# maggieHao/multi_modal_transformers_TokenMerge

Measured on NVIDIA B200. Metric: ToMe-transformer train samples/sec, higher is better.
Workload: dtype bf16

## Files before the change

multi_modal_transformers_tokenmerge_b200/csrc/attn_bwd.cu:

```cuda
#include <float.h>

#include "attn_meta.cuh"
#include "common.cuh"
#include "host_util.h"

namespace tome {

int check_attn_desc(const tome_attn_desc_t* d, const char* who);
int attn_generic_bwd(const tome_attn_desc_t* d, const tome_attn_grad_strides_t* gs, const void* q, const void* k, const void* v,
                     const void* out, const float* lse, const void* dout, void* dq, void* dk, void* dv, cudaStream_t stream);

constexpr int AB_D = 64;
constexpr int AB_THREADS = 192;
constexpr int DKT_SOFTMAX_WARPS = 8;
constexpr int DKT_THREADS = 320;
constexpr uint32_t AB_TMEM_COLS = 256;
constexpr int AB_MSLOTS = 3;

struct AttnBwdParams {
  int batch, tokens, heads, tp;
  float scale, scale_log2;
  const uint8_t* gid;
  const int32_t* pos;
  const uint8_t* meta;
  int store_ds;

  const float* size;
  const float* lse2;
  const float* delta;
  const uint8_t* keep_q;
  const uint8_t* keep_k;
  float inv_keep;
  __nv_bfloat16* dq; long long dq_bs, dq_ts;
  __nv_bfloat16* dk; long long dk_bs, dk_ts;
  __nv_bfloat16* dv; long long dv_bs, dv_ts;
  float* cs;
  long long cs_ld;
  int cs_q, cs_k, cs_v, n_t128;
};

__device__ __forceinline__ void warp_arrive(uint64_t* bar, int lane) {
  __syncwarp();
  if (lane == 0) mbar_arrive(bar);
}

__device__ __forceinline__ void ab_store_tile(uint8_t* stage, float* part, uint32_t tm_row, int rows_valid, __nv_bfloat16* gtile,
                                              long long row_stride, float* colsum_out, int bar) {
  const int tid = threadIdx.x & 127, row = tid, warp = tid >> 5, lane = tid & 31;
// ... 41 lines not shown
  const long long total = (long long)B * Tp * H * 8;
  if (idx < total) {
    const int ch = (int)(idx & 7);
    const long long r = idx >> 3;
    const int h = (int)(r % H);
    const long long bt = r / H;
    const int t = (int)(bt % Tp), b = (int)(bt / Tp);
    float s = 0.f;
    if (t < T) {
      const uint4 ov = __ldg(reinterpret_cast<const uint4*>(o + b * o_bs + t * o_ts + h * AB_D + ch * 8));
      const uint4 dv = __ldg(reinterpret_cast<const uint4*>(dout + b * do_bs + t * do_ts + h * AB_D + ch * 8));
      s = bf16_lo(ov.x) * bf16_lo(dv.x) + bf16_hi(ov.x) * bf16_hi(dv.x) + bf16_lo(ov.y) * bf16_lo(dv.y) +
          bf16_hi(ov.y) * bf16_hi(dv.y) + bf16_lo(ov.z) * bf16_lo(dv.z) + bf16_hi(ov.z) * bf16_hi(dv.z) +
          bf16_lo(ov.w) * bf16_lo(dv.w) + bf16_hi(ov.w) * bf16_hi(dv.w);
    }
    s += __shfl_xor_sync(0xffffffffu, s, 1);
    s += __shfl_xor_sync(0xffffffffu, s, 2);
    s += __shfl_xor_sync(0xffffffffu, s, 4);
    if (ch == 0) {
      const long long w = ((long long)b * H + h) * Tp + t;
      delta[w] = s;
      lse2[w] = t < T ? lse[((long long)b * H + h) * T + t] * 1.4426950408889634f : INFINITY;
    }
  }
}

constexpr int DKV_BK = 128;
constexpr int DKV_BQ = 64;
static_assert(DKV_BQ == ATTN_META_TILE, "query tiles and metadata tiles must coincide");
constexpr int DKV_KV_BYTES = DKV_BK * AB_D * 2;
constexpr int DKV_Q_BYTES = DKV_BQ * AB_D * 2;
constexpr int DKV_PT_BYTES = DKV_BK * DKV_BQ * 2;
constexpr int DKV_META_SLOT = 1280 + ATTN_DROP_TILE_BYTES;

constexpr int DKT_SMEM = 2 * DKV_KV_BYTES + 2 * 2 * DKV_Q_BYTES + 2 * DKV_PT_BYTES + AB_MSLOTS * DKV_META_SLOT + 256 + 1024;

template <bool DROP>
__global__ void __launch_bounds__(DKT_THREADS, 2)
attn_bwd_dkdv_ts_kernel(const __grid_constant__ CUtensorMap tm_q, const __grid_constant__ CUtensorMap tm_k,
                        const __grid_constant__ CUtensorMap tm_v, const __grid_constant__ CUtensorMap tm_do,
                        const __grid_constant__ CUtensorMap tm_ds, const AttnBwdParams p) {
  extern __shared__ uint8_t smem_raw[];
  uint8_t* smem = smem_raw + ((1024u - (smem_u32(smem_raw) & 1023u)) & 1023u);
  uint8_t* s_k = smem;
  uint8_t* s_v = s_k + DKV_KV_BYTES;
  uint8_t* s_qdo = s_v + DKV_KV_BYTES;
  uint8_t* s_dst = s_qdo + 2 * 2 * DKV_Q_BYTES;
  uint8_t* s_meta = s_dst + 2 * DKV_PT_BYTES;
  uint64_t* bars = reinterpret_cast<uint64_t*>(s_meta + AB_MSLOTS * DKV_META_SLOT);
  uint64_t* kv_full = bars;
  uint64_t* q_full = bars + 1;
  uint64_t* q_empty = bars + 3;
  uint64_t* s_full = bars + 5;
  uint64_t* dp_full = bars + 6;
  uint64_t* s_free = bars + 7;
  uint64_t* ps_ready = bars + 8;
  uint64_t* pd_free = bars + 9;
  uint64_t* meta_full = bars + 10;
  uint64_t* meta_empty = bars + 13;
  uint64_t* ds_stored = bars + 16;
  uint32_t* tmem_slot = reinterpret_cast<uint32_t*>(bars + 18);

  const int warp = threadIdx.x >> 5, lane = threadIdx.x & 31;
  const int kt = blockIdx.x, h = blockIdx.y, b = blockIdx.z;
  const int T = p.tokens;
  const int n_q = (T + DKV_BQ - 1) / DKV_BQ;
  const bool has_mask = p.gid != nullptr;

  if (threadIdx.x == 0) {
    mbar_init(kv_full, 1);
    for (int i = 0; i < 2; ++i) {
      mbar_init(&q_full[i], 1);
      mbar_init(&q_empty[i], 1);
    }
    mbar_init(s_full, 1);
    mbar_init(dp_full, 1);
    mbar_init(s_free, DKT_SOFTMAX_WARPS);
    mbar_init(ps_ready, DKT_SOFTMAX_WARPS);
    mbar_init(pd_free, 1);
    mbar_init(&ds_stored[0], 1);
    mbar_init(&ds_stored[1], 1);
    for (int i = 0; i < AB_MSLOTS; ++i) {
      mbar_init(&meta_full[i], 1);
      mbar_init(&meta_empty[i], DKT_SOFTMAX_WARPS);
    }
    fence_barrier_init();
  }
  if (warp == 8 && lane == 0) {
    tma_prefetch_desc(&tm_q);
    tma_prefetch_desc(&tm_k);
    tma_prefetch_desc(&tm_v);
    tma_prefetch_desc(&tm_do);
  }
  if (warp == 9) tmem_alloc(tmem_slot, AB_TMEM_COLS);
  tc_fence_before();
  __syncthreads();
  tc_fence_after();
  const uint32_t tmem_base = *tmem_slot;
  const uint32_t tm_st = tmem_base, tm_dpt = tmem_base + 64, tm_dk = tmem_base + 128, tm_dv = tmem_base + 192;
  auto tm_dsa = [&](int k) { return tm_dpt + (uint32_t)((k >> 1) * 32 + (k & 1) * 8); };
  auto tm_pa = [&](int k) { return tm_dpt + (uint32_t)((k >> 1) * 32 + 16 + (k & 1) * 8); };

  if (warp == 8) {
    if (lane == 0) {
      mbar_expect_tx(kv_full, 2 * DKV_KV_BYTES);
      tma_load_3d(s_k, &tm_k, kv_full, h * AB_D, kt * DKV_BK, b);
      tma_load_3d(s_v, &tm_v, kv_full, h * AB_D, kt * DKV_BK, b);
      const float* lse_row = p.lse2 + ((size_t)b * p.heads + h) * p.tp;
      const float* del_row = p.delta + ((size_t)b * p.heads + h) * p.tp;
      const uint8_t* meta_b = p.meta + (size_t)b * n_q * ATTN_META_BYTES;
      for (int i = 0; i < n_q; ++i) {
        const int ms = i % AB_MSLOTS;
        uint8_t* slot = s_meta + ms * DKV_META_SLOT;
        mbar_wait(&meta_empty[ms], ((i / AB_MSLOTS) & 1) ^ 1);
        mbar_expect_tx(&meta_full[ms], (has_mask ? 1280u : 512u) + (DROP ? ATTN_DROP_TILE_BYTES : 0));
        if constexpr (DROP) bulk_g2s(slot + 1280, p.keep_k + ((size_t)kt * n_q + i) * ATTN_DROP_TILE_BYTES, ATTN_DROP_TILE_BYTES, &meta_full[ms]);
        bulk_g2s(slot, lse_row + i * DKV_BQ, 256, &meta_full[ms]);
        bulk_g2s(slot + 256, del_row + i * DKV_BQ, 256, &meta_full[ms]);
        if (has_mask) bulk_g2s(slot + 512, meta_b + (size_t)i * ATTN_META_BYTES + ATTN_META_OFF_POS, 768, &meta_full[ms]);
        const int st = i & 1;
        mbar_wait(&q_empty[st], ((i >> 1) & 1) ^ 1);
        mbar_expect_tx(&q_full[st], 2 * DKV_Q_BYTES);
        tma_load_3d(s_qdo + st * 2 * DKV_Q_BYTES, &tm_q, &q_full[st], h * AB_D, i * DKV_BQ, b);
        tma_load_3d(s_qdo + st * 2 * DKV_Q_BYTES + DKV_Q_BYTES, &tm_do, &q_full[st], h * AB_D, i * DKV_BQ, b);
      }
    }
  } else if (warp == 9) {
    if (lane == 0) {
      constexpr uint32_t idesc_s = make_idesc_bf16(DKV_BK, DKV_BQ, false, false);
      constexpr uint32_t idesc_g = make_idesc_bf16(DKV_BK, AB_D, false, true);
      const uint32_t ak = smem_u32(s_k), av = smem_u32(s_v);
      mbar_wait(kv_full, 0);
      for (int i = 0; i <= n_q; ++i) {
        if (i < n_q) {
          const int st = i & 1;
          if (i >= 1) {
            mbar_wait(s_free, (i - 1) & 1);
            tc_fence_after();
          }
          mbar_wait(&q_full[st], (i >> 1) & 1);
          tc_fence_after();
          const uint32_t aq = smem_u32(s_qdo + st * 2 * DKV_Q_BYTES);
#pragma unroll
          for (int k = 0; k < AB_D / 16; ++k)
            umma_bf16(tm_st, make_smem_desc(ak + k * 32, 16, 1024), make_smem_desc(aq + k * 32, 16, 1024), idesc_s, k > 0);
          umma_commit(s_full);
        }
        if (i >= 1) {
          mbar_wait(ps_ready, (i - 1) & 1);
          tc_fence_after();
          const int st = (i - 1) & 1;
          const uint32_t aq = smem_u32(s_qdo + st * 2 * DKV_Q_BYTES), ado = aq + DKV_Q_BYTES;
          if (p.store_ds) {
            asm volatile("cp.async.bulk.tensor.3d.global.shared::cta.bulk_group [%0, {%2, %3, %4}], [%1];"
                         ::"l"(&tm_ds), "r"(smem_u32(s_dst + ((i - 1) & 1) * DKV_PT_BYTES)), "r"((i - 1) * DKV_BQ), "r"(kt * DKV_BK), "r"(b * p.heads + h) : "memory");
            asm volatile("cp.async.bulk.commit_group;" ::: "memory");
          }
#pragma unroll
          for (int k = 0; k < DKV_BQ / 16; ++k)
            umma_bf16_ts(tm_dv, tm_pa(k), make_smem_desc(ado + k * 2048, 8192, 1024), idesc_g, (i > 1 || k > 0) ? 1u : 0u);
#pragma unroll
          for (int k = 0; k < DKV_BQ / 16; ++k)
            umma_bf16_ts(tm_dk, tm_dsa(k), make_smem_desc(aq + k * 2048, 8192, 1024), idesc_g, (i > 1 || k > 0) ? 1u : 0u);
          umma_commit(pd_free);
          umma_commit(&q_empty[st]);
        }
        if (i < n_q) {
          const int st = i & 1;
          const uint32_t ado = smem_u32(s_qdo + st * 2 * DKV_Q_BYTES) + DKV_Q_BYTES;
#pragma unroll
          for (int k = 0; k < AB_D / 16; ++k)
            umma_bf16(tm_dpt, make_smem_desc(av + k * 32, 16, 1024), make_smem_desc(ado + k * 32, 16, 1024), idesc_s, k > 0);
          umma_commit(dp_full);
        }
        if (i >= 2 && p.store_ds) {
          asm volatile("cp.async.bulk.wait_group.read 1;" ::: "memory");
          mbar_arrive(&ds_stored[i & 1]);
        }
      }
      if (p.store_ds) asm volatile("cp.async.bulk.wait_group 0;" ::: "memory");
    }
  } else {
    const int row = (warp & 3) * 32 + lane;
    const int hq = warp >> 2;
    const int kk = kt * DKV_BK + row;
    const uint32_t lane_sel = ((uint32_t)((warp & 3) * 32)) << 16;
    const bool k_valid = kk < T;
    float bias2 = 0.f;
    int gk = 0, pk = 0;
    if (k_valid) {
      if (p.size) bias2 = log2f(p.size[(long long)b * T + kk]);
      if (has_mask) {
        gk = p.gid[(long long)b * T + kk];
        pk = p.pos[(long long)b * T + kk];
      }
    }
    const float2 scale2 = make_float2(p.scale_log2, p.scale_log2), bias22 = make_float2(bias2, bias2);
    const float2 sc2 = make_float2(p.scale, p.scale), ik2 = make_float2(p.inv_keep, p.inv_keep);
    const bool warp_active = kt * DKV_BK + (warp & 3) * 32 < T;
    uint8_t* dst_row0 = s_dst + row * 128;
    for (int i = 0; i < n_q; ++i) {
      const int ms = i % AB_MSLOTS;
      const uint8_t* slot = s_meta + ms * DKV_META_SLOT;
      mbar_wait(&meta_full[ms], (i / AB_MSLOTS) & 1);
      if (!warp_active) {
        mbar_wait(s_full, i & 1);
        tc_fence_before();
        warp_arrive(s_free, lane);
        mbar_wait(dp_full, i & 1);
        if (p.store_ds) {
          uint8_t* dst_row = dst_row0 + (i & 1) * DKV_PT_BYTES;
          if (i >= 2) mbar_wait(&ds_stored[i & 1], ((i - 2) >> 1) & 1);
#pragma unroll
          for (int ch = 0; ch < 4; ++ch) *reinterpret_cast<uint4*>(dst_row + ((hq * 4 + ch) << 4)) = make_uint4(0u, 0u, 0u, 0u);
          fence_proxy_async_smem();
        }
        warp_arrive(&meta_empty[ms], lane);
        tc_fence_before();
        warp_arrive(ps_ready, lane);
        continue;
      }
      uint32_t vw = 0xffffffffu;
      if (has_mask) {
        vw = *reinterpret_cast<const uint32_t*>(slot + 768 + gk * 8 + hq * 4);
        const uint32_t c = *reinterpret_cast<const uint32_t*>(slot + 1024 + gk * 8 + hq * 4);
        if (c) {
          const int* posq = reinterpret_cast<const int*>(slot + 512) + hq * 32;
          for (int q = 0; q < 32; ++q)
            if (((c >> q) & 1u) && pk <= posq[q]) vw |= 1u << q;
        }
      }
      if (!k_valid) vw = 0u;
      uint32_t kb = 0xffffffffu;
      if constexpr (DROP) kb = *reinterpret_cast<const uint32_t*>(slot + 1280 + row * 8 + hq * 4);
      const float4* lse4 = reinterpret_cast<const float4*>(slot) + hq * 8;
      const float4* del4 = reinterpret_cast<const float4*>(slot + 256) + hq * 8;
      uint32_t pe[16];
      mbar_wait(s_full, i & 1);
      tc_fence_after();
      {
        float sv[32];
        tmem_ld_f32x32(tm_st + lane_sel + hq * 32, sv);
        tmem_ld_wait();
        tc_fence_before();
        warp_arrive(s_free, lane);
#pragma unroll
        for (int c4 = 0; c4 < 8; ++c4) {
          const float4 l4 = lse4[c4];
#pragma unroll
          for (int u = 0; u < 2; ++u) {
            const int c = c4 * 4 + 2 * u;
            const float2 lv = u ? make_float2(l4.z, l4.w) : make_float2(l4.x, l4.y);
            float2 t = __ffma2_rn(make_float2(sv[c], sv[c + 1]), scale2, bias22);
            t = __fadd2_rn(t, make_float2(-lv.x, -lv.y));
            float2 e = make_float2(fast_exp2(t.x), fast_exp2(t.y));
            e.x = ((vw >> c) & 1u) ? e.x : 0.f;
            e.y = ((vw >> (c + 1)) & 1u) ? e.y : 0.f;
            pe[c >> 1] = pack_bf16(e.x, e.y);
          }
        }
      }
      uint32_t dw[16], pw[DROP ? 16 : 1];
      mbar_wait(dp_full, i & 1);
      tc_fence_after();
      {
        float dv[32];
        tmem_ld_f32x32(tm_dpt + lane_sel + hq * 32, dv);
        tmem_ld_wait();
#pragma unroll
        for (int c4 = 0; c4 < 8; ++c4) {
          const float4 d4 = del4[c4];
#pragma unroll
          for (int u = 0; u < 2; ++u) {
            const int c = c4 * 4 + 2 * u;
            const float2 dl = u ? make_float2(d4.z, d4.w) : make_float2(d4.x, d4.y);
            const uint32_t pwv = pe[c >> 1];
            const float2 pf = make_float2(bf16_lo(pwv), bf16_hi(pwv));
            float2 dp = make_float2(dv[c], dv[c + 1]);
            if constexpr (DROP) {
              const bool k0 = (kb >> c) & 1u, k1 = (kb >> (c + 1)) & 1u;
              dp = __fmul2_rn(dp, ik2);
              float2 pd = __fmul2_rn(pf, ik2);
              dp.x = k0 ? dp.x : 0.f; dp.y = k1 ? dp.y : 0.f;
              pd.x = k0 ? pd.x : 0.f; pd.y = k1 ? pd.y : 0.f;
              pw[c >> 1] = pack_bf16(pd.x, pd.y);
            }
            float2 g = __fadd2_rn(dp, make_float2(-dl.x, -dl.y));
            g = __fmul2_rn(g, sc2);
            g = __fmul2_rn(g, pf);
            dw[c >> 1] = pack_bf16(g.x, g.y);
          }
        }
      }
      tmem_st_x16(tm_dpt + lane_sel + hq * 32, dw);
      if constexpr (DROP) tmem_st_x16(tm_dpt + lane_sel + hq * 32 + 16, pw);
      else tmem_st_x16(tm_dpt + lane_sel + hq * 32 + 16, pe);
      if (p.store_ds) {
        uint8_t* dst_row = dst_row0 + (i & 1) * DKV_PT_BYTES;
        if (i >= 2) mbar_wait(&ds_stored[i & 1], ((i - 2) >> 1) & 1);
#pragma unroll
        for (int ch = 0; ch < 4; ++ch)
          *reinterpret_cast<uint4*>(dst_row + (((hq * 4 + ch) ^ (row & 7)) << 4)) = make_uint4(dw[4 * ch], dw[4 * ch + 1], dw[4 * ch + 2], dw[4 * ch + 3]);
        fence_proxy_async_smem();
      }
      tmem_st_wait();
      warp_arrive(&meta_empty[ms], lane);
      tc_fence_before();
      warp_arrive(ps_ready, lane);
    }
    mbar_wait(pd_free, (n_q - 1) & 1);
    tc_fence_after();
    {
      const int rows_valid = min(DKV_BK, T - kt * DKV_BK);
      float* cs_row = p.cs ? p.cs + ((long long)b * p.n_t128 + kt) * p.cs_ld + h * AB_D : nullptr;
      if (hq == 0)
        ab_store_tile(s_k, reinterpret_cast<float*>(s_qdo), tm_dk + lane_sel, rows_valid,
                      p.dk + (long long)b * p.dk_bs + (long long)kt * DKV_BK * p.dk_ts + h * AB_D, p.dk_ts, cs_row ? cs_row + p.cs_k : nullptr, 1);
      else
        ab_store_tile(s_v, reinterpret_cast<float*>(s_qdo) + 256, tm_dv + lane_sel, rows_valid,
                      p.dv + (long long)b * p.dv_bs + (long long)kt * DKV_BK * p.dv_ts + h * AB_D, p.dv_ts, cs_row ? cs_row + p.cs_v : nullptr, 2);
    }
  }
  tc_fence_before();
  __syncthreads();
  if (warp == 9) {
    tc_fence_after();
    tmem_dealloc(tmem_base, AB_TMEM_COLS);
  }
}

constexpr int DQ_BQ = 128;
constexpr int DQ_BK = 64;
static_assert(DQ_BK == ATTN_META_TILE, "key tiles and metadata tiles must coincide");
constexpr int DQ_Q_BYTES = DQ_BQ * AB_D * 2;
constexpr int DQ_K_BYTES = DQ_BK * AB_D * 2;
constexpr int DQ_DS_BYTES = DQ_BQ * DQ_BK * 2;
constexpr int DQ_META_SLOT = ATTN_META_KEY_BYTES + ATTN_DROP_TILE_BYTES;
constexpr int DQ_SMEM = 2 * DQ_Q_BYTES + 2 * 2 * DQ_K_BYTES + 2 * DQ_DS_BYTES + AB_MSLOTS * DQ_META_SLOT + 256 + 1024;

template <bool DROP>
__global__ void __launch_bounds__(AB_THREADS, 2)
attn_bwd_dq_kernel(const __grid_constant__ CUtensorMap tm_q, const __grid_constant__ CUtensorMap tm_k,
                   const __grid_constant__ CUtensorMap tm_v, const __grid_constant__ CUtensorMap tm_do,
                   const AttnBwdParams p) {
  extern __shared__ uint8_t smem_raw[];
  uint8_t* smem = smem_raw + ((1024u - (smem_u32(smem_raw) & 1023u)) & 1023u);
  uint8_t* s_q = smem;
  uint8_t* s_do = s_q + DQ_Q_BYTES;
  uint8_t* s_kv = s_do + DQ_Q_BYTES;
  uint8_t* s_ds = s_kv + 2 * 2 * DQ_K_BYTES;
  uint8_t* s_meta = s_ds + 2 * DQ_DS_BYTES;
  uint64_t* bars = reinterpret_cast<uint64_t*>(s_meta + AB_MSLOTS * DQ_META_SLOT);
  uint64_t* q_full = bars;
  uint64_t* kv_full = bars + 1;
  uint64_t* kv_empty = bars + 3;
  uint64_t* s_full = bars + 5;
  uint64_t* ds_ready = bars + 6;
  uint64_t* ds_free = bars + 7;
  uint64_t* meta_full = bars + 9;
  uint64_t* meta_empty = bars + 12;
// ... 357 lines not shown
    inv_keep = make_dropout(d->dropout_rate, d->dropout_seed, d->dropout_site).inv_keep;
  }
  {
    const long long total = (long long)B * Tp * H * 8;
    launch_k(attn_bwd_prep_kernel, (unsigned)((total + 255) / 256), 256, 0, stream, 
        B, T, Tp, H, reinterpret_cast<const __nv_bfloat16*>(out), d->o_batch_stride, d->o_token_stride,
        reinterpret_cast<const __nv_bfloat16*>(dout), gs->do_batch_stride, gs->do_token_stride, lse, ws.delta, ws.lse2);
    TOME_CUDA(cudaGetLastError());
  }
  const uint64_t hd = (uint64_t)H * d->head_dim;
  AttnBwdParams p;
  p.batch = B; p.tokens = T; p.heads = H; p.tp = Tp;
  p.scale = d->scale; p.scale_log2 = d->scale * 1.4426950408889634f;
  p.gid = d->gid; p.pos = d->pos; p.meta = ws.meta; p.size = d->size; p.lse2 = ws.lse2; p.delta = ws.delta;
  p.keep_q = keep_q; p.keep_k = keep_k; p.inv_keep = inv_keep;
  const bool from_ds = dq_from_ds(d);
  p.store_ds = from_ds ? 1 : 0;
  p.cs = gs->bias_partial; p.cs_ld = gs->bias_partial_ld;
  p.cs_q = gs->bias_q_col; p.cs_k = gs->bias_k_col; p.cs_v = gs->bias_v_col;
  p.n_t128 = ceil_div(T, 128);

  const uint64_t ds_tq = ((uint64_t)T + 7) / 8 * 8, ds_tk = (uint64_t)T;
  CUtensorMap tds_store, tds_load;
  if (from_ds) {
    if (int rc = make_tmap_3d_bf16(&tds_store, ws.ds, (uint64_t)T, ds_tk, (uint64_t)B * H, ds_tq, ds_tq * ds_tk, DKV_BK)) return rc;
    if (int rc = make_tmap_3d_bf16(&tds_load, ws.ds, (uint64_t)T, ds_tk, (uint64_t)B * H, ds_tq, ds_tq * ds_tk, DQG_BK)) return rc;
  } else {
    memset(&tds_store, 0, sizeof(tds_store));
  }
  p.dq = reinterpret_cast<__nv_bfloat16*>(dq); p.dq_bs = gs->dq_batch_stride; p.dq_ts = gs->dq_token_stride;
  p.dk = reinterpret_cast<__nv_bfloat16*>(dk); p.dk_bs = gs->dk_batch_stride; p.dk_ts = gs->dk_token_stride;
  p.dv = reinterpret_cast<__nv_bfloat16*>(dv); p.dv_bs = gs->dv_batch_stride; p.dv_ts = gs->dv_token_stride;
  static DynSmemOnce once[5];
  TOME_CUDA(ensure_dyn_smem(attn_bwd_dkdv_ts_kernel<false>, DKT_SMEM, once[0]));
  TOME_CUDA(ensure_dyn_smem(attn_bwd_dkdv_ts_kernel<true>, DKT_SMEM, once[1]));
  TOME_CUDA(ensure_dyn_smem(attn_bwd_dq_kernel<false>, DQ_SMEM, once[2]));
  TOME_CUDA(ensure_dyn_smem(attn_bwd_dq_kernel<true>, DQ_SMEM, once[3]));
  TOME_CUDA(ensure_dyn_smem(attn_bwd_dq_gemm_kernel, DQG_SMEM, once[4]));
  {
    CUtensorMap tq, tk, tv, tdo;
    if (int rc = make_tmap_3d_bf16(&tq, q, hd, T, B, d->q_token_stride, d->q_batch_stride, DKV_BQ)) return rc;
    if (int rc = make_tmap_3d_bf16(&tk, k, hd, T, B, d->k_token_stride, d->k_batch_stride, DKV_BK)) return rc;
    if (int rc = make_tmap_3d_bf16(&tv, v, hd, T, B, d->v_token_stride, d->v_batch_stride, DKV_BK)) return rc;
    if (int rc = make_tmap_3d_bf16(&tdo, dout, hd, T, B, gs->do_token_stride, gs->do_batch_stride, DKV_BQ)) return rc;
    dim3 grid(ceil_div(T, DKV_BK), H, B);
    if (keep_k) launch_k(attn_bwd_dkdv_ts_kernel<true>, grid, DKT_THREADS, DKT_SMEM, stream, tq, tk, tv, tdo, tds_store, p);
    else launch_k(attn_bwd_dkdv_ts_kernel<false>, grid, DKT_THREADS, DKT_SMEM, stream, tq, tk, tv, tdo, tds_store, p);
    TOME_CUDA(cudaGetLastError());
  }
  if (from_ds) {
    CUtensorMap tk;
    if (int rc = make_tmap_3d_bf16(&tk, k, hd, T, B, d->k_token_stride, d->k_batch_stride, DQG_BK)) return rc;
    dim3 grid(ceil_div(T, DQG_BQ), H, B);
    launch_k(attn_bwd_dq_gemm_kernel, grid, AB_THREADS, DQG_SMEM, stream, tds_load, tk, p);
    TOME_CUDA(cudaGetLastError());
  } else {
    CUtensorMap tq, tk, tv, tdo;
    if (int rc = make_tmap_3d_bf16(&tq, q, hd, T, B, d->q_token_stride, d->q_batch_stride, DQ_BQ)) return rc;
    if (int rc = make_tmap_3d_bf16(&tk, k, hd, T, B, d->k_token_stride, d->k_batch_stride, DQ_BK)) return rc;
    if (int rc = make_tmap_3d_bf16(&tv, v, hd, T, B, d->v_token_stride, d->v_batch_stride, DQ_BK)) return rc;
    if (int rc = make_tmap_3d_bf16(&tdo, dout, hd, T, B, gs->do_token_stride, gs->do_batch_stride, DQ_BQ)) return rc;
    dim3 grid(ceil_div(T, DQ_BQ), H, B);
    if (keep_q) launch_k(attn_bwd_dq_kernel<true>, grid, AB_THREADS, DQ_SMEM, stream, tq, tk, tv, tdo, p);
    else launch_k(attn_bwd_dq_kernel<false>, grid, AB_THREADS, DQ_SMEM, stream, tq, tk, tv, tdo, p);
    TOME_CUDA(cudaGetLastError());
  }
  return TOME_OK;
}
```

multi_modal_transformers_tokenmerge_b200/csrc/host_util.h:

```cpp
#pragma once
#include <cuda.h>
#include <cuda_runtime.h>
#include <stdarg.h>
#include <stdint.h>
#include <stdio.h>
#include <string.h>

#include <atomic>

#include "../../include/tome_b200.h"

namespace tome {

int set_error(int code, const char* fmt, ...);
void clear_error();

#define TOME_CHECK(cond, code, ...)                        \
  do {                                                     \
    if (!(cond)) return ::tome::set_error(code, __VA_ARGS__); \
  } while (0)

#define TOME_CUDA(expr)                                                                                   \
  do {                                                                                                    \
    cudaError_t _e = (expr);                                                                              \
// ... 16 lines not shown

struct Bump {
  uint8_t* base;
  size_t off = 0;
  size_t reserve(size_t bytes) {
    off = (off + 255) & ~size_t(255);
    const size_t at = off;
    off += bytes;
    return at;
  }
  template <typename T>
  T* take(size_t count) {
    const size_t at = reserve(count * sizeof(T));
    return base ? reinterpret_cast<T*>(base + at) : nullptr;
  }
  size_t total() const { return (off + 255) & ~size_t(255); }
};

struct DynSmemOnce {
  std::atomic<int> set[64];
};
template <typename Kernel>
inline cudaError_t ensure_dyn_smem(Kernel kernel, int bytes, DynSmemOnce& once) {
  int dev = 0;
  cudaError_t e = cudaGetDevice(&dev);
  if (e != cudaSuccess) return e;
  if (dev < 0 || dev >= 64) return cudaFuncSetAttribute(kernel, cudaFuncAttributeMaxDynamicSharedMemorySize, bytes);
  if (once.set[dev].load(std::memory_order_acquire) >= bytes) return cudaSuccess;
  e = cudaFuncSetAttribute(kernel, cudaFuncAttributeMaxDynamicSharedMemorySize, bytes);
  if (e == cudaSuccess) once.set[dev].store(bytes, std::memory_order_release);
  return e;
}

template <typename... KArgs, typename... Args>
inline cudaError_t launch_k(void (*kern)(KArgs...), dim3 grid, dim3 block, size_t smem, cudaStream_t stream, Args&&... args) {
  cudaLaunchConfig_t cfg;
  memset(&cfg, 0, sizeof(cfg));
  cfg.gridDim = grid;
  cfg.blockDim = block;
  cfg.dynamicSmemBytes = smem;
  cfg.stream = stream;
  return cudaLaunchKernelEx(&cfg, kern, static_cast<KArgs>(args)...);
}

enum ProfTag { PROF_GEMM = 0, PROF_ATTN_FWD, PROF_ATTN_BWD, PROF_MERGE_FWD, PROF_MERGE_BWD, PROF_SIM, PROF_SELECT,
               PROF_LN, PROF_COLSUM, PROF_OTHER, PROF_IMPORTANCE, PROF_PRUNE, PROF_NTAGS };
struct ProfScope {
  cudaStream_t st;
  bool rec;
  ProfScope(int tag, double work, int kernels, cudaStream_t stream);
  ~ProfScope();
};

}
```

Before: 7521.

## Make dK/dV attention backward kernel persistent with double-buffered TMEM accumulators

Converts the dK/dV backward kernel into a persistent kernel with one CTA per SM that loops over (key tile, head, batch) items. K/V tiles, S/dP tensor-memory tiles and the dK/dV accumulators are double-buffered, and dedicated epilogue warps store results while the next item computes. Q/dO staging is deepened to four stages. The goal is to hide per-tile prologue and epilogue and launch tail costs, at the price of halving occupancy, using 512 TMEM columns and adding more complex barrier choreography.

```diff
diff --git a/multi_modal_transformers_tokenmerge_b200/csrc/attn_bwd.cu b/multi_modal_transformers_tokenmerge_b200/csrc/attn_bwd.cu
--- a/multi_modal_transformers_tokenmerge_b200/csrc/attn_bwd.cu
+++ b/multi_modal_transformers_tokenmerge_b200/csrc/attn_bwd.cu
@@ -12,8 +12,6 @@
 
 constexpr int AB_D = 64;
 constexpr int AB_THREADS = 192;
-constexpr int DKT_SOFTMAX_WARPS = 8;
-constexpr int DKT_THREADS = 320;
 constexpr uint32_t AB_TMEM_COLS = 256;
 constexpr int AB_MSLOTS = 3;
 
@@ -121,300 +119,370 @@
 constexpr int DKV_Q_BYTES = DKV_BQ * AB_D * 2;
 constexpr int DKV_PT_BYTES = DKV_BK * DKV_BQ * 2;
 constexpr int DKV_META_SLOT = 1280 + ATTN_DROP_TILE_BYTES;
-
-constexpr int DKT_SMEM = 2 * DKV_KV_BYTES + 2 * 2 * DKV_Q_BYTES + 2 * DKV_PT_BYTES + AB_MSLOTS * DKV_META_SLOT + 256 + 1024;
+constexpr int DKV_QSTAGES = 4;
+constexpr int DKV_MSLOTS = 3;
+
+#ifndef DKT_GROUPS
+#define DKT_GROUPS 1
+#endif
+constexpr int DKT_SOFTMAX_GROUPS = DKT_GROUPS;
+constexpr int DKT_GROUP_WARPS = 8;
+constexpr int DKT_SOFTMAX_WARPS = DKT_SOFTMAX_GROUPS * DKT_GROUP_WARPS;
+constexpr int DKT_PRODUCER_WARP = DKT_SOFTMAX_WARPS, DKT_MMA_WARP = DKT_SOFTMAX_WARPS + 1;
+constexpr int DKT_EPI_WARP0 = DKT_SOFTMAX_WARPS + 2;
+constexpr int DKT_THREADS = (DKT_EPI_WARP0 + 4) * 32;
+constexpr uint32_t DKT_TMEM_COLS = 512;
+constexpr int DKT_NBARS = 2 + 2 + 2 * DKV_QSTAGES + 2 + 2 + 2 + 2 + 2 + 2 + 2 * DKV_MSLOTS + 2;
+constexpr int DKT_SMEM = 2 * 2 * DKV_KV_BYTES
+                         + DKV_QSTAGES * 2 * DKV_Q_BYTES
+                         + 2 * DKV_PT_BYTES
+                         + 2 * DKV_KV_BYTES
+                         + DKV_MSLOTS * DKV_META_SLOT + 2 * 1024
+                         + DKT_NBARS * 8 + 8 + 1024;
+static_assert(2 * (DKT_SMEM + 1024) > 228 * 1024, "the dK/dV kernel must run one CTA per SM");
+static_assert(DKT_SMEM <= 227 * 1024, "dK/dV kernel shared memory");
 
 template <bool DROP>
-__global__ void __launch_bounds__(DKT_THREADS, 2)
-attn_bwd_dkdv_ts_kernel(const __grid_constant__ CUtensorMap tm_q, const __grid_constant__ CUtensorMap tm_k,
-                        const __grid_constant__ CUtensorMap tm_v, const __grid_constant__ CUtensorMap tm_do,
-                        const __grid_constant__ CUtensorMap tm_ds, const AttnBwdParams p) {
+__global__ void __launch_bounds__(DKT_THREADS, 1)
+attn_bwd_dkdv_kernel(const __grid_constant__ CUtensorMap tm_q, const __grid_constant__ CUtensorMap tm_k,
+                     const __grid_constant__ CUtensorMap tm_v, const __grid_constant__ CUtensorMap tm_do,
+                     const __grid_constant__ CUtensorMap tm_ds, const AttnBwdParams p) {
   extern __shared__ uint8_t smem_raw[];
   uint8_t* smem = smem_raw + ((1024u - (smem_u32(smem_raw) & 1023u)) & 1023u);
-  uint8_t* s_k = smem;
-  uint8_t* s_v = s_k + DKV_KV_BYTES;
-  uint8_t* s_qdo = s_v + DKV_KV_BYTES;
-  uint8_t* s_dst = s_qdo + 2 * 2 * DKV_Q_BYTES;
-  uint8_t* s_meta = s_dst + 2 * DKV_PT_BYTES;
-  uint64_t* bars = reinterpret_cast<uint64_t*>(s_meta + AB_MSLOTS * DKV_META_SLOT);
+  uint8_t* s_kv = smem;
+  uint8_t* s_qdo = s_kv + 2 * 2 * DKV_KV_BYTES;
+  uint8_t* s_dst = s_qdo + DKV_QSTAGES * 2 * DKV_Q_BYTES;
+  uint8_t* s_ep = s_dst + 2 * DKV_PT_BYTES;
+  uint8_t* s_meta = s_ep + 2 * DKV_KV_BYTES;
+  float* s_part = reinterpret_cast<float*>(s_meta + DKV_MSLOTS * DKV_META_SLOT);
+  uint64_t* bars = reinterpret_cast<uint64_t*>(s_part + 512);
   uint64_t* kv_full = bars;
-  uint64_t* q_full = bars + 1;
-  uint64_t* q_empty = bars + 3;
-  uint64_t* s_full = bars + 5;
-  uint64_t* dp_full = bars + 6;
-  uint64_t* s_free = bars + 7;
-  uint64_t* ps_ready = bars + 8;
-  uint64_t* pd_free = bars + 9;
-  uint64_t* meta_full = bars + 10;
-  uint64_t* meta_empty = bars + 13;
-  uint64_t* ds_stored = bars + 16;
-  uint32_t* tmem_slot = reinterpret_cast<uint32_t*>(bars + 18);
+  uint64_t* kv_empty = kv_full + 2;
+  uint64_t* q_full = kv_empty + 2;
+  uint64_t* q_empty = q_full + DKV_QSTAGES;
+  uint64_t* s_full = q_empty + DKV_QSTAGES;
+  uint64_t* dp_full = s_full + 2;
+  uint64_t* s_free = dp_full + 2;
+  uint64_t* ps_ready = s_free + 2;
+  uint64_t* acc_full = ps_ready + 2;
+  uint64_t* acc_empty = acc_full + 2;
+  uint64_t* meta_full = acc_empty + 2;
+  uint64_t* meta_empty = meta_full + DKV_MSLOTS;
+  uint64_t* ds_stored = meta_empty + DKV_MSLOTS;
+  uint32_t* tmem_slot = reinterpret_cast<uint32_t*>(ds_stored + 2);
 
   const int warp = threadIdx.x >> 5, lane = threadIdx.x & 31;
-  const int kt = blockIdx.x, h = blockIdx.y, b = blockIdx.z;
   const int T = p.tokens;
   const int n_q = (T + DKV_BQ - 1) / DKV_BQ;
+  const int n_kt = (T + DKV_BK - 1) / DKV_BK;
+  const int n_items = (p.batch * p.heads * n_kt - (int)blockIdx.x + (int)gridDim.x - 1) / (int)gridDim.x;
   const bool has_mask = p.gid != nullptr;
+  auto item = [&](int n, int& kt, int& h, int& b) {
+    const int it = (int)blockIdx.x + n * (int)gridDim.x;
+    kt = it % n_kt;
+    const int bh = it / n_kt;
+    h = bh % p.heads;
+    b = bh / p.heads;
+  };
 
   if (threadIdx.x == 0) {
-    mbar_init(kv_full, 1);
     for (int i = 0; i < 2; ++i) {
+      mbar_init(&kv_full[i], 1);
+      mbar_init(&kv_empty[i], 1);
+      mbar_init(&s_full[i], 1);
+      mbar_init(&dp_full[i], 1);
+      mbar_init(&s_free[i], DKT_GROUP_WARPS);
+      mbar_init(&ps_ready[i], DKT_GROUP_WARPS);
+      mbar_init(&acc_full[i], 1);
+      mbar_init(&acc_empty[i], 4);
+      mbar_init(&ds_stored[i], 1);
+    }
+    for (int i = 0; i < DKV_QSTAGES; ++i) {
       mbar_init(&q_full[i], 1);
       mbar_init(&q_empty[i], 1);
     }
-    mbar_init(s_full, 1);
-    mbar_init(dp_full, 1);
-    mbar_init(s_free, DKT_SOFTMAX_WARPS);
-    mbar_init(ps_ready, DKT_SOFTMAX_WARPS);
-    mbar_init(pd_free, 1);
-    mbar_init(&ds_stored[0], 1);
-    mbar_init(&ds_stored[1], 1);
-    for (int i = 0; i < AB_MSLOTS; ++i) {
+    for (int i = 0; i < DKV_MSLOTS; ++i) {
       mbar_init(&meta_full[i], 1);
-      mbar_init(&meta_empty[i], DKT_SOFTMAX_WARPS);
+      mbar_init(&meta_empty[i], DKT_GROUP_WARPS);
     }
     fence_barrier_init();
   }
-  if (warp == 8 && lane == 0) {
+  if (warp == DKT_PRODUCER_WARP && lane == 0) {
     tma_prefetch_desc(&tm_q);
     tma_prefetch_desc(&tm_k);
     tma_prefetch_desc(&tm_v);
     tma_prefetch_desc(&tm_do);
   }
-  if (warp == 9) tmem_alloc(tmem_slot, AB_TMEM_COLS);
+  if (warp == DKT_MMA_WARP) tmem_alloc(tmem_slot, DKT_TMEM_COLS);
   tc_fence_before();
   __syncthreads();
   tc_fence_after();
   const uint32_t tmem_base = *tmem_slot;
-  const uint32_t tm_st = tmem_base, tm_dpt = tmem_base + 64, tm_dk = tmem_base + 128, tm_dv = tmem_base + 192;
-  auto tm_dsa = [&](int k) { return tm_dpt + (uint32_t)((k >> 1) * 32 + (k & 1) * 8); };
-  auto tm_pa = [&](int k) { return tm_dpt + (uint32_t)((k >> 1) * 32 + 16 + (k & 1) * 8); };
-
-  if (warp == 8) {
+  auto tm_st = [&](int s) { return tmem_base + 64u * (uint32_t)s; };
+  auto tm_dpt = [&](int s) { return tmem_base + 128u + 64u * (uint32_t)s; };
+  auto tm_dk = [&](int a) { return tmem_base + 256u + 128u * (uint32_t)a; };
+  auto tm_dv = [&](int a) { return tmem_base + 320u + 128u * (uint32_t)a; };
+
+  if (warp == DKT_PRODUCER_WARP) {
     if (lane == 0) {
-      mbar_expect_tx(kv_full, 2 * DKV_KV_BYTES);
-      tma_load_3d(s_k, &tm_k, kv_full, h * AB_D, kt * DKV_BK, b);
-      tma_load_3d(s_v, &tm_v, kv_full, h * AB_D, kt * DKV_BK, b);
-      const float* lse_row = p.lse2 + ((size_t)b * p.heads + h) * p.tp;
-      const float* del_row = p.delta + ((size_t)b * p.heads + h) * p.tp;
-      const uint8_t* meta_b = p.meta + (size_t)b * n_q * ATTN_META_BYTES;
-      for (int i = 0; i < n_q; ++i) {
-        const int ms = i % AB_MSLOTS;
-        uint8_t* slot = s_meta + ms * DKV_META_SLOT;
-        mbar_wait(&meta_empty[ms], ((i / AB_MSLOTS) & 1) ^ 1);
-        mbar_expect_tx(&meta_full[ms], (has_mask ? 1280u : 512u) + (DROP ? ATTN_DROP_TILE_BYTES : 0));
-        if constexpr (DROP) bulk_g2s(slot + 1280, p.keep_k + ((size_t)kt * n_q + i) * ATTN_DROP_TILE_BYTES, ATTN_DROP_TILE_BYTES, &meta_full[ms]);
-        bulk_g2s(slot, lse_row + i * DKV_BQ, 256, &meta_full[ms]);
-        bulk_g2s(slot + 256, del_row + i * DKV_BQ, 256, &meta_full[ms]);
-        if (has_mask) bulk_g2s(slot + 512, meta_b + (size_t)i * ATTN_META_BYTES + ATTN_META_OFF_POS, 768, &meta_full[ms]);
-        const int st = i & 1;
-        mbar_wait(&q_empty[st], ((i >> 1) & 1) ^ 1);
-        mbar_expect_tx(&q_full[st], 2 * DKV_Q_BYTES);
-        tma_load_3d(s_qdo + st * 2 * DKV_Q_BYTES, &tm_q, &q_full[st], h * AB_D, i * DKV_BQ, b);
-        tma_load_3d(s_qdo + st * 2 * DKV_Q_BYTES + DKV_Q_BYTES, &tm_do, &q_full[st], h * AB_D, i * DKV_BQ, b);
-      }
-    }
-  } else if (warp == 9) {
+      for (int n = 0, g = 0; n < n_items; ++n) {
+        int kt, h, b;
+        item(n, kt, h, b);
+        const int kb = n & 1;
+        mbar_wait(&kv_empty[kb], ((n >> 1) & 1) ^ 1);
+        mbar_expect_tx(&kv_full[kb], 2 * DKV_KV_BYTES);
+        tma_load_3d(s_kv + kb * 2 * DKV_KV_BYTES, &tm_k, &kv_full[kb], h * AB_D, kt * DKV_BK, b);
+        tma_load_3d(s_kv + kb * 2 * DKV_KV_BYTES + DKV_KV_BYTES, &tm_v, &kv_full[kb], h * AB_D, kt * DKV_BK, b);
+        const float* lse_row = p.lse2 + ((size_t)b * p.heads + h) * p.tp;
+        const float* del_row = p.delta + ((size_t)b * p.heads + h) * p.tp;
+        const uint8_t* meta_b = p.meta + (size_t)b * n_q * ATTN_META_BYTES;
+        for (int i = 0; i < n_q; ++i, ++g) {
+          const int ms = g % DKV_MSLOTS;
+          uint8_t* slot = s_meta + ms * DKV_META_SLOT;
+          mbar_wait(&meta_empty[ms], ((g / DKV_MSLOTS) & 1) ^ 1);
+          mbar_expect_tx(&meta_full[ms], (has_mask ? 1280u : 512u) + (DROP ? ATTN_DROP_TILE_BYTES : 0));
+          if constexpr (DROP) bulk_g2s(slot + 1280, p.keep_k + ((size_t)kt * n_q + i) * ATTN_DROP_TILE_BYTES, ATTN_DROP_TILE_BYTES, &meta_full[ms]);
+          bulk_g2s(slot, lse_row + i * DKV_BQ, 256, &meta_full[ms]);
+          bulk_g2s(slot + 256, del_row + i * DKV_BQ, 256, &meta_full[ms]);
+          if (has_mask) bulk_g2s(slot + 512, meta_b + (size_t)i * ATTN_META_BYTES + ATTN_META_OFF_POS, 768, &meta_full[ms]);
+          const int st = g % DKV_QSTAGES;
+          mbar_wait(&q_empty[st], ((g / DKV_QSTAGES) & 1) ^ 1);
+          mbar_expect_tx(&q_full[st], 2 * DKV_Q_BYTES);
+          tma_load_3d(s_qdo + st * 2 * DKV_Q_BYTES, &tm_q, &q_full[st], h * AB_D, i * DKV_BQ, b);
+          tma_load_3d(s_qdo + st * 2 * DKV_Q_BYTES + DKV_Q_BYTES, &tm_do, &q_full[st], h * AB_D, i * DKV_BQ, b);
+        }
+      }
+    }
+  } else if (warp == DKT_MMA_WARP) {
     if (lane == 0) {
       constexpr uint32_t idesc_s = make_idesc_bf16(DKV_BK, DKV_BQ, false, false);
       constexpr uint32_t idesc_g = make_idesc_bf16(DKV_BK, AB_D, false, true);
-      const uint32_t ak = smem_u32(s_k), av = smem_u32(s_v);
-      mbar_wait(kv_full, 0);
-      for (int i = 0; i <= n_q; ++i) {
-        if (i < n_q) {
-          const int st = i & 1;
-          if (i >= 1) {
-            mbar_wait(s_free, (i - 1) & 1);
+      const int G = n_items * n_q;
+      for (int g = 0; g <= G; ++g) {
+        if (g < G) {
+          const int n = g / n_q, i = g - n * n_q, sb = g & 1, st = g % DKV_QSTAGES, kb = n & 1;
+          if (i == 0) {
+            mbar_wait(&kv_full[kb], (n >> 1) & 1);
             tc_fence_after();
           }
-          mbar_wait(&q_full[st], (i >> 1) & 1);
+          if (g >= 2) {
+            mbar_wait(&s_free[sb], ((g - 2) >> 1) & 1);
+            tc_fence_after();
+          }
+          mbar_wait(&q_full[st], (g / DKV_QSTAGES) & 1);
           tc_fence_after();
-          const uint32_t aq = smem_u32(s_qdo + st * 2 * DKV_Q_BYTES);
+          const uint32_t ak = smem_u32(s_kv + kb * 2 * DKV_KV_BYTES), av = ak + DKV_KV_BYTES;
+          const uint32_t aq = smem_u32(s_qdo + st * 2 * DKV_Q_BYTES), ado = aq + DKV_Q_BYTES;
 #pragma unroll
           for (int k = 0; k < AB_D / 16; ++k)
-            umma_bf16(tm_st, make_smem_desc(ak + k * 32, 16, 1024), make_smem_desc(aq + k * 32, 16, 1024), idesc_s, k > 0);
-          umma_commit(s_full);
-        }
-        if (i >= 1) {
-          mbar_wait(ps_ready, (i - 1) & 1);
+            umma_bf16(tm_st(sb), make_smem_desc(ak + k * 32, 16, 1024), make_smem_desc(aq + k * 32, 16, 1024), idesc_s, k > 0);
+          umma_commit(&s_full[sb]);
+#pragma unroll
+          for (int k = 0; k < AB_D / 16; ++k)
+            umma_bf16(tm_dpt(sb), make_smem_desc(av + k * 32, 16, 1024), make_smem_desc(ado + k * 32, 16, 1024), idesc_s, k > 0);
+          umma_commit(&dp_full[sb]);
+          if (i == n_q - 1) umma_commit(&kv_empty[kb]);
+          if (g >= 2 && p.store_ds) {
+            asm volatile("cp.async.bulk.wait_group.read 0;" ::: "memory");
+            mbar_arrive(&ds_stored[sb]);
+          }
+        }
+        if (g >= 1) {
+          const int g1 = g - 1, n = g1 / n_q, i = g1 - n * n_q, sb = g1 & 1, st = g1 % DKV_QSTAGES, ab = n & 1;
+          mbar_wait(&ps_ready[sb], (g1 >> 1) & 1);
           tc_fence_after();
-          const int st = (i - 1) & 1;
+          if (i == 0) {
+            mbar_wait(&acc_empty[ab], ((n >> 1) & 1) ^ 1);
+            tc_fence_after();
+          }
           const uint32_t aq = smem_u32(s_qdo + st * 2 * DKV_Q_BYTES), ado = aq + DKV_Q_BYTES;
           if (p.store_ds) {
+            int kt, h, b;
+            item(n, kt, h, b);
             asm volatile("cp.async.bulk.tensor.3d.global.shared::cta.bulk_group [%0, {%2, %3, %4}], [%1];"
-                         ::"l"(&tm_ds), "r"(smem_u32(s_dst + ((i - 1) & 1) * DKV_PT_BYTES)), "r"((i - 1) * DKV_BQ), "r"(kt * DKV_BK), "r"(b * p.heads + h) : "memory");
+                         ::"l"(&tm_ds), "r"(smem_u32(s_dst + sb * DKV_PT_BYTES)), "r"(i * DKV_BQ), "r"(kt * DKV_BK), "r"(b * p.heads + h) : "memory");
             asm volatile("cp.async.bulk.commit_group;" ::: "memory");
           }
 #pragma unroll
           for (int k = 0; k < DKV_BQ / 16; ++k)
-            umma_bf16_ts(tm_dv, tm_pa(k), make_smem_desc(ado + k * 2048, 8192, 1024), idesc_g, (i > 1 || k > 0) ? 1u : 0u);
+            umma_bf16_ts(tm_dv(ab), tm_dpt(sb) + (uint32_t)((k >> 1) * 32 + 16 + (k & 1) * 8),
+                         make_smem_desc(ado + k * 2048, 8192, 1024), idesc_g, (i > 0 || k > 0) ? 1u : 0u);
 #pragma unroll
           for (int k = 0; k < DKV_BQ / 16; ++k)
-            umma_bf16_ts(tm_dk, tm_dsa(k), make_smem_desc(aq + k * 2048, 8192, 1024), idesc_g, (i > 1 || k > 0) ? 1u : 0u);
-          umma_commit(pd_free);
+            umma_bf16_ts(tm_dk(ab), tm_dpt(sb) + (uint32_t)((k >> 1) * 32 + (k & 1) * 8),
+                         make_smem_desc(aq + k * 2048, 8192, 1024), idesc_g, (i > 0 || k > 0) ? 1u : 0u);
           umma_commit(&q_empty[st]);
-        }
-        if (i < n_q) {
-          const int st = i & 1;
-          const uint32_t ado = smem_u32(s_qdo + st * 2 * DKV_Q_BYTES) + DKV_Q_BYTES;
-#pragma unroll
-          for (int k = 0; k < AB_D / 16; ++k)
-            umma_bf16(tm_dpt, make_smem_desc(av + k * 32, 16, 1024), make_smem_desc(ado + k * 32, 16, 1024), idesc_s, k > 0);
-          umma_commit(dp_full);
-        }
-        if (i >= 2 && p.store_ds) {
-          asm volatile("cp.async.bulk.wait_group.read 1;" ::: "memory");
-          mbar_arrive(&ds_stored[i & 1]);
+          if (i == n_q - 1) umma_commit(&acc_full[ab]);
         }
       }
       if (p.store_ds) asm volatile("cp.async.bulk.wait_group 0;" ::: "memory");
     }
-  } else {
+  } else if (warp < DKT_SOFTMAX_WARPS) {
     const int row = (warp & 3) * 32 + lane;
-    const int hq = warp >> 2;
-    const int kk = kt * DKV_BK + row;
+    const int hq = (warp >> 2) & 1;
+    const int group = warp / DKT_GROUP_WARPS;
     const uint32_t lane_sel = ((uint32_t)((warp & 3) * 32)) << 16;
-    const bool k_valid = kk < T;
-    float bias2 = 0.f;
-    int gk = 0, pk = 0;
-    if (k_valid) {
-      if (p.size) bias2 = log2f(p.size[(long long)b * T + kk]);
-      if (has_mask) {
-        gk = p.gid[(long long)b * T + kk];
-        pk = p.pos[(long long)b * T + kk];
-      }
-    }
-    const float2 scale2 = make_float2(p.scale_log2, p.scale_log2), bias22 = make_float2(bias2, bias2);
+    const float2 scale2 = make_float2(p.scale_log2, p.scale_log2);
     const float2 sc2 = make_float2(p.scale, p.scale), ik2 = make_float2(p.inv_keep, p.inv_keep);
-    const bool warp_active = kt * DKV_BK + (warp & 3) * 32 < T;
-    uint8_t* dst_row0 = s_dst + row * 128;
-    for (int i = 0; i < n_q; ++i) {
-      const int ms = i % AB_MSLOTS;
-      const uint8_t* slot = s_meta + ms * DKV_META_SLOT;
-      mbar_wait(&meta_full[ms], (i / AB_MSLOTS) & 1);
-      if (!warp_active) {
-        mbar_wait(s_full, i & 1);
-        tc_fence_before();
-        warp_arrive(s_free, lane);
-        mbar_wait(dp_full, i & 1);
+    struct KeyRow { float bias2; int gk, pk; };
+    auto key_row = [&](int n) {
+      KeyRow r{0.f, 0, 0};
+      if (n < n_items) {
+        int kt, h, b;
+        item(n, kt, h, b);
+        const int kk = kt * DKV_BK + row;
+        if (kk < T) {
+          if (p.size) r.bias2 = log2f(p.size[(long long)b * T + kk]);
+          if (has_mask) {
+            r.gk = p.gid[(long long)b * T + kk];
+            r.pk = p.pos[(long long)b * T + kk];
+          }
+        }
+      }
+      return r;
+    };
+    KeyRow next = key_row(0);
+    for (int n = 0, g = 0; n < n_items; ++n) {
+      int kt, h, b;
+      item(n, kt, h, b);
+      const KeyRow key = next;
+      next = key_row(n + 1);
+      const bool k_valid = kt * DKV_BK + row < T;
+      const float2 bias22 = make_float2(key.bias2, key.bias2);
+      const bool warp_active = kt * DKV_BK + (warp & 3) * 32 < T;
+      for (int i = 0; i < n_q; ++i, ++g) {
+        if (g % DKT_SOFTMAX_GROUPS != group) continue;
+        const int ms = g % DKV_MSLOTS, sb = g & 1;
+        const uint8_t* slot = s_meta + ms * DKV_META_SLOT;
+        uint8_t* dst_row = s_dst + sb * DKV_PT_BYTES + row * 128;
+        mbar_wait(&meta_full[ms], (g / DKV_MSLOTS) & 1);
+        if (!warp_active) {
+          mbar_wait(&s_full[sb], (g >> 1) & 1);
+          tc_fence_before();
+          warp_arrive(&s_free[sb], lane);
+          mbar_wait(&dp_full[sb], (g >> 1) & 1);
+          if (p.store_ds) {
+            if (g >= 2) mbar_wait(&ds_stored[sb], ((g - 2) >> 1) & 1);
+#pragma unroll
+            for (int ch = 0; ch < 4; ++ch) *reinterpret_cast<uint4*>(dst_row + ((hq * 4 + ch) << 4)) = make_uint4(0u, 0u, 0u, 0u);
+            fence_proxy_async_smem();
+          }
+          warp_arrive(&meta_empty[ms], lane);
+          tc_fence_before();
+          warp_arrive(&ps_ready[sb], lane);
+          continue;
+        }
+        uint32_t vw = 0xffffffffu;
+        if (has_mask) {
+          vw = *reinterpret_cast<const uint32_t*>(slot + 768 + key.gk * 8 + hq * 4);
+          const uint32_t c = *reinterpret_cast<const uint32_t*>(slot + 1024 + key.gk * 8 + hq * 4);
+          if (c) {
+            const int* posq = reinterpret_cast<const int*>(slot + 512) + hq * 32;
+            for (int q = 0; q < 32; ++q)
+              if (((c >> q) & 1u) && key.pk <= posq[q]) vw |= 1u << q;
+          }
+        }
+        if (!k_valid) vw = 0u;
+        uint32_t kb = 0xffffffffu;
+        if constexpr (DROP) kb = *reinterpret_cast<const uint32_t*>(slot + 1280 + row * 8 + hq * 4);
+        const float4* lse4 = reinterpret_cast<const float4*>(slot) + hq * 8;
+        const float4* del4 = reinterpret_cast<const float4*>(slot + 256) + hq * 8;
+        uint32_t pe[16];
+        mbar_wait(&s_full[sb], (g >> 1) & 1);
+        tc_fence_after();
+        {
+          float sv[32];
+          tmem_ld_f32x32(tm_st(sb) + lane_sel + hq * 32, sv);
+          tmem_ld_wait();
+          tc_fence_before();
+          warp_arrive(&s_free[sb], lane);
+#pragma unroll
+          for (int c4 = 0; c4 < 8; ++c4) {
+            const float4 l4 = lse4[c4];
+#pragma unroll
+            for (int u = 0; u < 2; ++u) {
+              const int c = c4 * 4 + 2 * u;
+              const float2 lv = u ? make_float2(l4.z, l4.w) : make_float2(l4.x, l4.y);
+              float2 t = __ffma2_rn(make_float2(sv[c], sv[c + 1]), scale2, bias22);
+              t = __fadd2_rn(t, make_float2(-lv.x, -lv.y));
+              float2 e = make_float2(fast_exp2(t.x), fast_exp2(t.y));
+              e.x = ((vw >> c) & 1u) ? e.x : 0.f;
+              e.y = ((vw >> (c + 1)) & 1u) ? e.y : 0.f;
+              pe[c >> 1] = pack_bf16(e.x, e.y);
+            }
+          }
+        }
+        uint32_t dw[16], pw[DROP ? 16 : 1];
+        mbar_wait(&dp_full[sb], (g >> 1) & 1);
+        tc_fence_after();
+        {
+          float dv[32];
+          tmem_ld_f32x32(tm_dpt(sb) + lane_sel + hq * 32, dv);
+          tmem_ld_wait();
+#pragma unroll
+          for (int c4 = 0; c4 < 8; ++c4) {
+            const float4 d4 = del4[c4];
+#pragma unroll
+            for (int u = 0; u < 2; ++u) {
+              const int c = c4 * 4 + 2 * u;
+              const float2 dl = u ? make_float2(d4.z, d4.w) : make_float2(d4.x, d4.y);
+              const uint32_t pwv = pe[c >> 1];
+              const float2 pf = make_float2(bf16_lo(pwv), bf16_hi(pwv));
+              float2 dp = make_float2(dv[c], dv[c + 1]);
+              if constexpr (DROP) {
+                const bool k0 = (kb >> c) & 1u, k1 = (kb >> (c + 1)) & 1u;
+                dp = __fmul2_rn(dp, ik2);
+                float2 pd = __fmul2_rn(pf, ik2);
+                dp.x = k0 ? dp.x : 0.f; dp.y = k1 ? dp.y : 0.f;
+                pd.x = k0 ? pd.x : 0.f; pd.y = k1 ? pd.y : 0.f;
+                pw[c >> 1] = pack_bf16(pd.x, pd.y);
+              }
+              float2 gr = __fadd2_rn(dp, make_float2(-dl.x, -dl.y));
+              gr = __fmul2_rn(gr, sc2);
+              gr = __fmul2_rn(gr, pf);
+              dw[c >> 1] = pack_bf16(gr.x, gr.y);
+            }
+          }
+        }
+        tmem_st_x16(tm_dpt(sb) + lane_sel + hq * 32, dw);
+        if constexpr (DROP) tmem_st_x16(tm_dpt(sb) + lane_sel + hq * 32 + 16, pw);
+        else tmem_st_x16(tm_dpt(sb) + lane_sel + hq * 32 + 16, pe);
         if (p.store_ds) {
-          uint8_t* dst_row = dst_row0 + (i & 1) * DKV_PT_BYTES;
-          if (i >= 2) mbar_wait(&ds_stored[i & 1], ((i - 2) >> 1) & 1);
-#pragma unroll
-          for (int ch = 0; ch < 4; ++ch) *reinterpret_cast<uint4*>(dst_row + ((hq * 4 + ch) << 4)) = make_uint4(0u, 0u, 0u, 0u);
+          if (g >= 2) mbar_wait(&ds_stored[sb], ((g - 2) >> 1) & 1);
+#pragma unroll
+          for (int ch = 0; ch < 4; ++ch)
+            *reinterpret_cast<uint4*>(dst_row + (((hq * 4 + ch) ^ (row & 7)) << 4)) = make_uint4(dw[4 * ch], dw[4 * ch + 1], dw[4 * ch + 2], dw[4 * ch + 3]);
           fence_proxy_async_smem();
         }
+        tmem_st_wait();
         warp_arrive(&meta_empty[ms], lane);
         tc_fence_before();
-        warp_arrive(ps_ready, lane);
-        continue;
-      }
-      uint32_t vw = 0xffffffffu;
-      if (has_mask) {
-        vw = *reinterpret_cast<const uint32_t*>(slot + 768 + gk * 8 + hq * 4);
-        const uint32_t c = *reinterpret_cast<const uint32_t*>(slot + 1024 + gk * 8 + hq * 4);
-        if (c) {
-          const int* posq = reinterpret_cast<const int*>(slot + 512) + hq * 32;
-          for (int q = 0; q < 32; ++q)
-            if (((c >> q) & 1u) && pk <= posq[q]) vw |= 1u << q;
-        }
-      }
-      if (!k_valid) vw = 0u;
-      uint32_t kb = 0xffffffffu;
-      if constexpr (DROP) kb = *reinterpret_cast<const uint32_t*>(slot + 1280 + row * 8 + hq * 4);
-      const float4* lse4 = reinterpret_cast<const float4*>(slot) + hq * 8;
-      const float4* del4 = reinterpret_cast<const float4*>(slot + 256) + hq * 8;
-      uint32_t pe[16];
-      mbar_wait(s_full, i & 1);
+        warp_arrive(&ps_ready[sb], lane);
+      }
+    }
+  } else if (warp >= DKT_EPI_WARP0) {
+    const uint32_t lane_sel = ((uint32_t)((warp & 3) * 32)) << 16;
+    for (int n = 0; n < n_items; ++n) {
+      int kt, h, b;
+      item(n, kt, h, b);
+      const int ab = n & 1;
+      mbar_wait(&acc_full[ab], (n >> 1) & 1);
       tc_fence_after();
-      {
-        float sv[32];
-        tmem_ld_f32x32(tm_st + lane_sel + hq * 32, sv);
-        tmem_ld_wait();
-        tc_fence_before();
-        warp_arrive(s_free, lane);
-#pragma unroll
-        for (int c4 = 0; c4 < 8; ++c4) {
-          const float4 l4 = lse4[c4];
-#pragma unroll
-          for (int u = 0; u < 2; ++u) {
-            const int c = c4 * 4 + 2 * u;
-            const float2 lv = u ? make_float2(l4.z, l4.w) : make_float2(l4.x, l4.y);
-            float2 t = __ffma2_rn(make_float2(sv[c], sv[c + 1]), scale2, bias22);
-            t = __fadd2_rn(t, make_float2(-lv.x, -lv.y));
-            float2 e = make_float2(fast_exp2(t.x), fast_exp2(t.y));
-            e.x = ((vw >> c) & 1u) ? e.x : 0.f;
-            e.y = ((vw >> (c + 1)) & 1u) ? e.y : 0.f;
-            pe[c >> 1] = pack_bf16(e.x, e.y);
-          }
-        }
-      }
-      uint32_t dw[16], pw[DROP ? 16 : 1];
-      mbar_wait(dp_full, i & 1);
-      tc_fence_after();
-      {
-        float dv[32];
-        tmem_ld_f32x32(tm_dpt + lane_sel + hq * 32, dv);
-        tmem_ld_wait();
-#pragma unroll
-        for (int c4 = 0; c4 < 8; ++c4) {
-          const float4 d4 = del4[c4];
-#pragma unroll
-          for (int u = 0; u < 2; ++u) {
-            const int c = c4 * 4 + 2 * u;
-            const float2 dl = u ? make_float2(d4.z, d4.w) : make_float2(d4.x, d4.y);
-            const uint32_t pwv = pe[c >> 1];
-            const float2 pf = make_float2(bf16_lo(pwv), bf16_hi(pwv));
-            float2 dp = make_float2(dv[c], dv[c + 1]);
-            if constexpr (DROP) {
-              const bool k0 = (kb >> c) & 1u, k1 = (kb >> (c + 1)) & 1u;
-              dp = __fmul2_rn(dp, ik2);
-              float2 pd = __fmul2_rn(pf, ik2);
-              dp.x = k0 ? dp.x : 0.f; dp.y = k1 ? dp.y : 0.f;
-              pd.x = k0 ? pd.x : 0.f; pd.y = k1 ? pd.y : 0.f;
-              pw[c >> 1] = pack_bf16(pd.x, pd.y);
-            }
-            float2 g = __fadd2_rn(dp, make_float2(-dl.x, -dl.y));
-            g = __fmul2_rn(g, sc2);
-            g = __fmul2_rn(g, pf);
-            dw[c >> 1] = pack_bf16(g.x, g.y);
-          }
-        }
-      }
-      tmem_st_x16(tm_dpt + lane_sel + hq * 32, dw);
-      if constexpr (DROP) tmem_st_x16(tm_dpt + lane_sel + hq * 32 + 16, pw);
-      else tmem_st_x16(tm_dpt + lane_sel + hq * 32 + 16, pe);
-      if (p.store_ds) {
-        uint8_t* dst_row = dst_row0 + (i & 1) * DKV_PT_BYTES;
-        if (i >= 2) mbar_wait(&ds_stored[i & 1], ((i - 2) >> 1) & 1);
-#pragma unroll
-        for (int ch = 0; ch < 4; ++ch)
-          *reinterpret_cast<uint4*>(dst_row + (((hq * 4 + ch) ^ (row & 7)) << 4)) = make_uint4(dw[4 * ch], dw[4 * ch + 1], dw[4 * ch + 2], dw[4 * ch + 3]);
-        fence_proxy_async_smem();
-      }
-      tmem_st_wait();
-      warp_arrive(&meta_empty[ms], lane);
-      tc_fence_before();
-      warp_arrive(ps_ready, lane);
-    }
-    mbar_wait(pd_free, (n_q - 1) & 1);
-    tc_fence_after();
-    {
       const int rows_valid = min(DKV_BK, T - kt * DKV_BK);
       float* cs_row = p.cs ? p.cs + ((long long)b * p.n_t128 + kt) * p.cs_ld + h * AB_D : nullptr;
-      if (hq == 0)
-        ab_store_tile(s_k, reinterpret_cast<float*>(s_qdo), tm_dk + lane_sel, rows_valid,
-                      p.dk + (long long)b * p.dk_bs + (long long)kt * DKV_BK * p.dk_ts + h * AB_D, p.dk_ts, cs_row ? cs_row + p.cs_k : nullptr, 1);
-      else
-        ab_store_tile(s_v, reinterpret_cast<float*>(s_qdo) + 256, tm_dv + lane_sel, rows_valid,
-                      p.dv + (long long)b * p.dv_bs + (long long)kt * DKV_BK * p.dv_ts + h * AB_D, p.dv_ts, cs_row ? cs_row + p.cs_v : nullptr, 2);
+      ab_store_tile(s_ep, s_part, tm_dk(ab) + lane_sel, rows_valid,
+                    p.dk + (long long)b * p.dk_bs + (long long)kt * DKV_BK * p.dk_ts + h * AB_D, p.dk_ts, cs_row ? cs_row + p.cs_k : nullptr, 1);
+      ab_store_tile(s_ep + DKV_KV_BYTES, s_part + 256, tm_dv(ab) + lane_sel, rows_valid,
+                    p.dv + (long long)b * p.dv_bs + (long long)kt * DKV_BK * p.dv_ts + h * AB_D, p.dv_ts, cs_row ? cs_row + p.cs_v : nullptr, 1);
+      tc_fence_before();
+      warp_arrive(&acc_empty[ab], lane);
     }
   }
   tc_fence_before();
   __syncthreads();
-  if (warp == 9) {
+  if (warp == DKT_MMA_WARP) {
     tc_fence_after();
-    tmem_dealloc(tmem_base, AB_TMEM_COLS);
+    tmem_dealloc(tmem_base, DKT_TMEM_COLS);
   }
 }
 
@@ -838,8 +906,8 @@
   p.dk = reinterpret_cast<__nv_bfloat16*>(dk); p.dk_bs = gs->dk_batch_stride; p.dk_ts = gs->dk_token_stride;
   p.dv = reinterpret_cast<__nv_bfloat16*>(dv); p.dv_bs = gs->dv_batch_stride; p.dv_ts = gs->dv_token_stride;
   static DynSmemOnce once[5];
-  TOME_CUDA(ensure_dyn_smem(attn_bwd_dkdv_ts_kernel<false>, DKT_SMEM, once[0]));
-  TOME_CUDA(ensure_dyn_smem(attn_bwd_dkdv_ts_kernel<true>, DKT_SMEM, once[1]));
+  TOME_CUDA(ensure_dyn_smem(attn_bwd_dkdv_kernel<false>, DKT_SMEM, once[0]));
+  TOME_CUDA(ensure_dyn_smem(attn_bwd_dkdv_kernel<true>, DKT_SMEM, once[1]));
   TOME_CUDA(ensure_dyn_smem(attn_bwd_dq_kernel<false>, DQ_SMEM, once[2]));
   TOME_CUDA(ensure_dyn_smem(attn_bwd_dq_kernel<true>, DQ_SMEM, once[3]));
   TOME_CUDA(ensure_dyn_smem(attn_bwd_dq_gemm_kernel, DQG_SMEM, once[4]));
@@ -849,9 +917,12 @@
     if (int rc = make_tmap_3d_bf16(&tk, k, hd, T, B, d->k_token_stride, d->k_batch_stride, DKV_BK)) return rc;
     if (int rc = make_tmap_3d_bf16(&tv, v, hd, T, B, d->v_token_stride, d->v_batch_stride, DKV_BK)) return rc;
     if (int rc = make_tmap_3d_bf16(&tdo, dout, hd, T, B, gs->do_token_stride, gs->do_batch_stride, DKV_BQ)) return rc;
-    dim3 grid(ceil_div(T, DKV_BK), H, B);
-    if (keep_k) launch_k(attn_bwd_dkdv_ts_kernel<true>, grid, DKT_THREADS, DKT_SMEM, stream, tq, tk, tv, tdo, tds_store, p);
-    else launch_k(attn_bwd_dkdv_ts_kernel<false>, grid, DKT_THREADS, DKT_SMEM, stream, tq, tk, tv, tdo, tds_store, p);
+    int sms = 0;
+    TOME_CUDA(device_sm_count(&sms));
+    const int items = ceil_div(T, DKV_BK) * H * B;
+    const dim3 grid((unsigned)(items < sms ? items : sms));
+    if (keep_k) launch_k(attn_bwd_dkdv_kernel<true>, grid, DKT_THREADS, DKT_SMEM, stream, tq, tk, tv, tdo, tds_store, p);
+    else launch_k(attn_bwd_dkdv_kernel<false>, grid, DKT_THREADS, DKT_SMEM, stream, tq, tk, tv, tdo, tds_store, p);
     TOME_CUDA(cudaGetLastError());
   }
   if (from_ds) {
diff --git a/multi_modal_transformers_tokenmerge_b200/csrc/host_util.h b/multi_modal_transformers_tokenmerge_b200/csrc/host_util.h
--- a/multi_modal_transformers_tokenmerge_b200/csrc/host_util.h
+++ b/multi_modal_transformers_tokenmerge_b200/csrc/host_util.h
@@ -72,6 +72,18 @@
   return e;
 }
 
+inline cudaError_t device_sm_count(int* out) {
+  static std::atomic<int> cached[64];
+  int dev = 0;
+  cudaError_t e = cudaGetDevice(&dev);
+  if (e != cudaSuccess) return e;
+  const bool cache = dev >= 0 && dev < 64;
+  if (cache && (*out = cached[dev].load(std::memory_order_acquire)) > 0) return cudaSuccess;
+  e = cudaDeviceGetAttribute(out, cudaDevAttrMultiProcessorCount, dev);
+  if (e == cudaSuccess && cache) cached[dev].store(*out, std::memory_order_release);
+  return e;
+}
+
 template <typename... KArgs, typename... Args>
 inline cudaError_t launch_k(void (*kern)(KArgs...), dim3 grid, dim3 block, size_t smem, cudaStream_t stream, Args&&... args) {
   cudaLaunchConfig_t cfg;
```

After: 7318, median of 6. -2.7%, worse.
